# theouterlimitz/Python-Audio-Mastering

Hardware: AMD Instinct MI355X
Metric: stereo frames/sec through full mastering chain, 44.1 kHz f32; 1/2/4/8 GPU (higher is better)
Workload: dtype f64; 1 GPU; C2: 5-min 44.1 kHz stereo f32 track per GPU, full chain (sat 30, techno EQ, width 1.3, multiband defaults, LUFS -14); frames_per_track=13230000, tracks_per_gpu=1, frames_per_rank_step=13230000, parallelism=file-sharded x1, in=f32 interleaved (decoded PCM16), out=f32 interleaved

## Files before the change

### include/mastering.h

```cpp
#ifndef MASTERING_AMD_H
#define MASTERING_AMD_H

#include <stdint.h>

#ifdef __cplusplus
extern "C" {
#endif

#define MM_OK 0
#define MM_ERR_ARG (-1)
#define MM_ERR_HIP (-2)
#define MM_ERR_RCCL (-3)
#define MM_ERR_STATE (-4)

#define MM_MAX_DIM 8
#define MM_TILE_POW 8
#define MM_BLK_POW 65

#define MM_OUT_I16 0
#define MM_OUT_F32 1

#define MM_IN_F32 0
#define MM_IN_I16 1
#define MM_IN_I24 2
// ... 142 lines not shown
    const struct mm_job *loud;
} mm_delivery;

typedef struct mm_solve_geom {
    int32_t tps;
    int32_t tile_rows;
    int32_t rows;
    int32_t walk_block;
    int64_t cols_per_chunk;
    int64_t chunks;
    int64_t chunk_plane_bytes;
    int64_t plane_bytes;
    int32_t col_block;
    int32_t rms_group_tiles;
} mm_solve_geom;

int mm_create(int device, mm_ctx **ctx);
int mm_destroy(mm_ctx *ctx);
const char *mm_last_error(mm_ctx *ctx);
int mm_sync(mm_ctx *ctx);
#define MM_ABI_VERSION 5
int mm_version(void);
int mm_solve_geometry(const mm_job *job, mm_solve_geom *out);
const char *mm_source_sha(void);

int mm_master(mm_ctx *ctx, const mm_job *job, const void *in, void *out, mm_result *res);
int mm_master_device(mm_ctx *ctx, const mm_job *job, const void *d_in, void *d_out, mm_result *res);

#define MM_BATCH_STREAMS 8
int mm_master_batch(mm_ctx *ctx, int n, const mm_job *jobs, const void *const *d_in, void *const *d_out,
                    mm_result *res);

int mm_meter_device(mm_ctx *ctx, const void *d_pcm, int kind, int64_t frames, int channels, const mm_job *loud,
                    mm_meter *out);
int mm_meter_pcm(mm_ctx *ctx, const void *pcm, int kind, int64_t frames, int channels, const mm_job *loud,
                 mm_meter *out);
int mm_last_meters(mm_ctx *ctx, int cap, mm_meter *out);
int mm_true_peak_host(const int16_t *pcm, int64_t frames, int channels, mm_meter *out);
int mm_meter_span(void);

int mm_r128_from_hops(const double *e, int64_t hops, int32_t rate, mm_r128 *out);
int mm_r128_host(const int16_t *pcm, int64_t frames, int channels, int32_t rate, const double sos[2][5],
                 double *hops_out, int64_t hops_cap, mm_r128 *out);
int mm_r128_device(mm_ctx *ctx, const void *d_pcm, int kind, int64_t frames, int channels, int32_t rate,
                   const double sos[2][5], mm_r128 *out);
int mm_r128_pcm(mm_ctx *ctx, const void *pcm, int kind, int64_t frames, int channels, int32_t rate,
// ... 102 lines not shown
```

### python-audio-mastering_amd/csrc/common.h

```cpp
#pragma once
#include <hip/hip_runtime.h>
#include <stdint.h>

#pragma clang fp contract(off)

namespace mm {

__device__ __forceinline__ void lds_barrier() { asm volatile("s_waitcnt lgkmcnt(0)\n\ts_barrier" ::: "memory"); }

__device__ __forceinline__ int32_t pair_swap(int32_t v) { return __builtin_amdgcn_mov_dpp(v, 0xB1, 0xF, 0xF, true); }
__device__ __forceinline__ double pair_swap(double v) {
    const int64_t b = __double_as_longlong(v);
    const int32_t lo = pair_swap((int32_t)(b & 0xffffffff)), hi = pair_swap((int32_t)(b >> 32));
    return __longlong_as_double(((int64_t)hi << 32) | (uint32_t)lo);
}

__device__ __forceinline__ float sqrt_f32_cr(float x) { return (float)__dsqrt_rn((double)x); }

template <int B, int NB, typename V, typename LD, typename PROC>
__device__ __forceinline__ void stream(int len, LD &&ld, PROC &&proc) {
    constexpr int R = B * NB;
    if (len <= 0) return;
    V buf[NB][B];
#pragma unroll
// ... 38 lines not shown
    return true;
}

struct CompArgs {
    int64_t N_proc, G;
    int T, K, ch, warmup;
    int TPS;
    int64_t SPC;
    int64_t GS;
    const short2 *band[3];
    const double *lut[3];
    uint32_t r0[3];
    int look[3];
    double attack_frames[3], release_frames[3];
    double rcp_attack[3], rcp_release[3];
    double *Ms[3];
    int TP;
    int RP;
    int64_t chunk_elems;
    const double *E[3], *tail[3];
    int32_t *cnt[3];
    double *mmax[3];
    double *ced[3];
    int32_t *total[3];
    int32_t *cbtot[3];
    int32_t *rank[3];
    int32_t *nact[3];
    int32_t *tl[3];
    double *mmaxc[3];
    double *cedc[3];
    double *tstc[3];
    double *descc[3];
    double *start[3];
    double *end[3];
    uint32_t *claim[3];
    int jumps;
    int sjump;
    double *sdesc[3];
    int32_t *se0[3];
    uint32_t stamp;
    int heads;
    int e_tiles;
    unsigned int *changed;
    unsigned long long *walked;
    uint32_t *trace;
    int sweep_idx;
// ... 21 lines not shown
```

### python-audio-mastering_amd/csrc/compressor.hip

```cpp
#include "common.h"
#include "lookback.h"

namespace mm {

template <bool V>
struct BoolTag {
    static constexpr bool value = V;
};

__device__ __forceinline__ double div_cr(double m, double d, double rd) {
    const double q = m * rd;
    const double rem = fma(-q, d, m);
    return fma(rem, rd, q);
}

#ifndef MM_RMS_NB
#define MM_RMS_NB 3
#endif
constexpr int RMS_B = 8;
constexpr int RMS_TPS = 4;

__device__ __forceinline__ void tile_col(const CompArgs &a, int64_t g, int64_t *s, int *k) {
    const int64_t c = g / a.K, j = g - c * a.K;
    *s = c * a.SPC + j / a.TPS;
    *k = (int)(j - (j / a.TPS) * a.TPS);
}
__device__ __forceinline__ uint32_t col_elem(const CompArgs &a, int64_t s) {
    const int64_t sl = s % a.SPC;
    return (uint32_t)((sl >> 6) * (int64_t)a.RP * 64 + (sl & 63));
}
__device__ __forceinline__ double *chunk_plane(const CompArgs &a, int b, int64_t c) {
    return a.Ms[b] + c * a.chunk_elems;
}

#ifndef MM_RMS_MINB
#define MM_RMS_MINB 1
#endif
__device__ __forceinline__ uint32_t rms_exact1(double S, double n, float inv_b) {
    int32_t r = (int32_t)__builtin_amdgcn_sqrtf((float)S * inv_b);
    const double rd = (double)(r + 1);
// ... 87 lines not shown
            r = rms_exact1(S, n, inv);
            S += (double)frame_energy2(p.in) - (double)frame_energy2(p.drop);
        } else {
            r = n > 0.0 ? rms_exact1(S, n, inv) : 0u;
            const bool drops = i_proc >= skip;
            S += (double)frame_energy2(p.in) - (drops ? (double)frame_energy2(p.drop) : 0.0);
            if (!drops) {
                n += ch;
                inv = rcp_biased(n);
            }
            ++i_proc;
        }
        active += r >= r0 ? 1 : 0;
        rmx = max(rmx, r);
        return r;
    };
    const int jB = lane & 7;
    const int tlC = lane * 4 + w;
    const int64_t jtC = jt0 + tlC, gC = cc * a.K + jtC;
    const bool vC = jtC < a.K && gC < a.G;
    double *Mo = chunk_plane(a, b, cc);
    uint32_t eC = col_elem(a, cc * a.SPC + jtC / 4) + (uint32_t)(w * a.TP) * 64u;
    double ce = 0.0, De = 0.0;
    const int slotC = w * 68 + lane;

    constexpr int B = RMS_B, NB = MM_RMS_NB;
    const int NBK = (T + B - 1) / B;
    const int NBKP = (NBK + NB - 1) / NB * NB;
    Pair buf[NB][B];
    double gm[B];
#pragma unroll
    for (int j = 0; j < B; ++j) gm[j] = 0.0;
    auto issue_gathers = [&](int q) __attribute__((always_inline)) {
        asm volatile("" ::: "memory");
#pragma unroll
        for (int r8 = 0; r8 < B; ++r8) {
            const int tl = w * 64 + r8 * 8 + (lane >> 3);
            gm[r8] = lut[Rs[q & 1][jB][tl]];
        }
    };
    auto finish_gathers = [&](int q) __attribute__((always_inline)) {
#pragma unroll
        for (int r8 = 0; r8 < B; ++r8) {
            const int tl = w * 64 + r8 * 8 + (lane >> 3);
            Mst[q & 1][jB][rt_slot(tl)] = gm[r8];
        }
    };
    const __amdgpu_buffer_rsrc_t Mr =
        __builtin_amdgcn_make_buffer_rsrc(Mo, (short)0, (int)(a.chunk_elems * 8), 0x00020000);
    constexpr uint32_t DROP = 0xFFFFFFF0u;
    typedef unsigned int u32x2 __attribute__((ext_vector_type(2)));
    auto phase_c = [&](int q) __attribute__((always_inline)) {
        const int nv = q >= 0 ? max(min(B, T - q * B), 0) : 0;
        double m[B];
#pragma unroll
        for (int j = 0; j < B; ++j) m[j] = Mst[q & 1][j][slotC];
#pragma unroll
        for (int j = 0; j < B; ++j) {
            const uint32_t off = (vC && j < nv) ? (eC + (uint32_t)j * 64u) * 8u : DROP;
            __builtin_amdgcn_raw_buffer_store_b64(__builtin_bit_cast(u32x2, m[j]), Mr, off, 0, 0);
        }
        eC += (uint32_t)nv * 64u;
#pragma unroll
        for (int j = 0; j < B; ++j) {
            const double mj = j < nv ? m[j] : 0.0;
            const double d = div_cr(mj, Rf, rR);
            ce = vmax(mj, ce - d);
            De += d;
        }
    };
    auto run = [&](auto st, auto &&load) __attribute__((always_inline)) {
#pragma unroll
        for (int k = 0; k < NB; ++k) {
#pragma unroll
            for (int j = 0; j < B; ++j) buf[k][j] = load(k * B + j);
            __builtin_amdgcn_sched_barrier(0);
        }
        auto body = [&](int k, int q) __attribute__((always_inline)) {
            uint32_t r[B];
            const int nvA = lenA - q * B;
#pragma unroll
            for (int j = 0; j < B; ++j) r[j] = j < nvA ? rms_step(buf[k][j], st) : 0u;
#pragma unroll
            for (int j = 0; j < B; ++j) buf[k][j] = load((q + NB) * B + j);
#pragma unroll
            for (int j = 0; j < B; ++j) Rs[q & 1][j][tlA] = (uint16_t)r[j];
            finish_gathers(q - 1);
            issue_gathers(q);
            __syncthreads();
            phase_c(q - 1);
        };
        for (int q0 = 0; q0 < NBKP; q0 += NB) {
#pragma unroll
            for (int k = 0; k < NB; ++k) body(k, q0 + k);
        }
    };
    if (!__any(vA)) run(BoolTag<true>{}, [](int) { return Pair{make_short2(0, 0), make_short2(0, 0)}; });
    else if (steady) run(BoolTag<true>{}, ld_steady);
    else run(BoolTag<false>{}, ld);
    finish_gathers(NBKP - 1);
    __syncthreads();
    phase_c(NBKP - 1);
    if (vC)
        for (int i = T; i < a.TP; ++i, eC += 64u) Mo[eC] = 0.0;
    if (vC) reinterpret_cast<double2 *>(a.ced[b])[gC] = make_double2(ce, De);
    if (vA) {
        a.cnt[b][gA] = active;
        a.mmax[b][gA] = lut[rmx];
    }
    {
        const int na = (int)__popcll(__ballot(vA && active != 0));
        if (lane == 0 && na) atomicAdd(a.cbtot[b] + cbk, na);
    }
    int v = vA ? active : 0;
    for (int o = 32; o > 0; o >>= 1) v += __shfl_xor(v, o);
    if (lane == 0 && v) atomicAdd(a.total[b] + cc, v);
}

__global__ void __launch_bounds__(64) comp_trim_kernel(CompArgs a, const int64_t *pad) {
    const int b = blockIdx.y, lane = threadIdx.x, T = a.T;
    const int64_t e = pad[2 * blockIdx.x], nx = pad[2 * blockIdx.x + 1];
    int v = 0;
    for (int64_t g = e / T + lane; g < nx / T; g += 64) {
        const int c = a.cnt[b][g];
        const int first = (int)max((int64_t)0, e - g * T);
        if (c == 0) continue;
        if (first == 0) {
            v += c;
// ... 1 lines not shown
        }
        int64_t s;
        int k;
        tile_col(a, g, &s, &k);
        const double *M = chunk_plane(a, b, g / a.K) + col_elem(a, s) + (uint32_t)(k * a.TP) * 64u;
        for (int n = first; n < T; ++n) v += M[(uint32_t)n * 64u] != 0.0 ? 1 : 0;
    }
    for (int o = 32; o > 0; o >>= 1) v += __shfl_xor(v, o);
    if (lane == 0 && v) atomicSub(a.total[b] + (nx / ((int64_t)T * a.K) - 1), v);
}

struct BandStep {
    double A, R, rA, rR;
};

__device__ __forceinline__ BandStep band_step(const CompArgs &a, int b) {
    BandStep s;
    s.A = a.attack_frames[b];
    s.R = a.release_frames[b];
    s.rA = a.rcp_attack[b];
    s.rR = a.rcp_release[b];
    return s;
}

__device__ __forceinline__ int binade(double x) { return (int)((uint64_t)__double_as_longlong(x) >> 52) - 1023; }


__device__ __forceinline__ double vmin(double x, double y) {
    double r;
    asm("v_min_f64 %0, %1, %2" : "=v"(r) : "v"(x), "v"(y));
    return r;
}

__device__ __forceinline__ double lean_step(double att, double m, double inc, double dec) {
    const double up = vmin(att + inc, m);
    const double dn = att - dec;
    return att <= m ? up : dn;
}

struct Super {
    int64_t ci0;
    int ntiles;
    bool first;
    bool last;
};

__device__ __forceinline__ Super super_of_na(const CompArgs &a, int64_t s, int na) {
    Super r;
// ... 109 lines not shown
    BandStep bs;
    double *tst;
    int i0, nst;
    __device__ __forceinline__ void init(const double (&m)[WB]) {
#pragma unroll
        for (int k = 0; k < WP; ++k) {
            inc[k] = div_cr(m[k], bs.A, bs.rA);
            dec[k] = div_cr(m[k], bs.R, bs.rR);
        }
    }
    __device__ __forceinline__ void tile(int i) {
        if (ST && i >= i0 && i < i0 + nst) tst[i - i0] = att;
        if (i == i0) sv = att;
        if (i == i0 + nst) out = att;
    }
    __device__ __forceinline__ void frame(int j, double m, double ma) {
        const double ik = inc[j % WP], dk = dec[j % WP];
        inc[j % WP] = div_cr(ma, bs.A, bs.rA);
        dec[j % WP] = div_cr(ma, bs.R, bs.rR);
        att = lean_step(att, m, ik, dk);
    }
};

#ifndef MM_JB
#define MM_JB 8
#endif
constexpr int JB = MM_JB;
constexpr int JF = JB < 4 ? JB : 4;
struct SegDesc {
    double mx;
    int e0;
    double q[2 * JB];
};
constexpr int DREC = 2 * JB;

__device__ __forceinline__ bool release_jump(const SegDesc &d, double att, double *out) {
    constexpr uint64_t MANT = (1ull << 52) - 1;
    const uint64_t ab = (uint64_t)__double_as_longlong(att);
    const int k = (int)(ab >> 52) - 1023 - d.e0;
    if (!(att > 0.0) || k < 0 || k >= JB) return false;
    const int idx = 2 * k + (int)(ab & 1);
    double q = d.q[0];
#pragma unroll
    for (int j = 1; j < 2 * JB; ++j) q = idx == j ? d.q[j] : q;
    const double x = att - q;
    const uint64_t xb = (uint64_t)__double_as_longlong(x);
    if (!(x > d.mx) || (xb >> 52) != (ab >> 52) || (xb & MANT) == 0) return false;
    *out = x;
    return true;
}

struct Describer {
    static constexpr uint64_t MANT = (1ull << 52) - 1;
    double r0[2 * JB], r[2 * JB];
    int e0;
    BandStep bs;
    __device__ __forceinline__ void init(const double (&)[WB]) {}
    __device__ __forceinline__ void tile(int i) {
        if (i != 0) return;
#pragma unroll
        for (int k = 0; k < 2 * JB; ++k) {
            const uint64_t bits = ((uint64_t)(e0 + k / 2 + 1023) << 52) | (MANT - 63 + (uint64_t)(k % 2));
            r0[k] = r[k] = __longlong_as_double((long long)bits);
        }
    }
    __device__ __forceinline__ void frame(int, double m, double) {
        const double dec = div_cr(m, bs.R, bs.rR);
#pragma unroll
        for (int k = 0; k < 2 * JB; ++k) r[k] = r[k] - dec;
    }
    __device__ __forceinline__ void store(double *rec_) const {
        double2 *rec = reinterpret_cast<double2 *>(rec_);
        double q[2 * JB];
#pragma unroll
        for (int k = 0; k < 2 * JB; ++k) {
            const uint64_t rb = (uint64_t)__double_as_longlong(r[k]);
            const bool ok = (rb >> 52) == (uint64_t)(e0 + k / 2 + 1023) && (rb & MANT) != 0;
            q[k] = ok ? r0[k] - r[k] : __longlong_as_double(0x7ff8000000000000ll);
        }
#pragma unroll
        for (int k = 0; k < JB; ++k) rec[k] = make_double2(q[2 * k], q[2 * k + 1]);
    }
};

#ifndef MM_DESC_NB
#define MM_DESC_NB 1
#endif
constexpr int DESC_MAX_TPS = 8;

__global__ void __launch_bounds__(64 * DESC_MAX_TPS) comp_describe_kernel(CompArgs a) {
    __shared__ int32_t wsum[DESC_MAX_TPS], base_s;
    __shared__ uint8_t flag[64 * DESC_MAX_TPS];
    __shared__ int32_t pre[64 * DESC_MAX_TPS];
    const int b = blockIdx.y;
    const int TPS = a.TPS, NT = 64 * TPS;
    const int kc = threadIdx.x >> 6, l = threadIdx.x & 63;
    const int64_t cb = blockIdx.x;
    const int64_t sc = cb * 64 + l;
    const int64_t cc = sc / a.SPC;
    const int64_t cbl = (sc - cc * a.SPC) >> 6;
    const int64_t jt = (sc - cc * a.SPC) * TPS + kc;
    const int64_t g = cc * a.K + jt;
    const bool valid = jt < a.K && g < a.G;
    const bool live = valid && a.cnt[b][g] != 0;
    flag[l * TPS + kc] = live ? 1 : 0;
    if (threadIdx.x < 64) {
        int32_t acc = 0;
        const int32_t *ct = a.cbtot[b] + cc * (a.SPC >> 6);
        for (int64_t q = threadIdx.x; q < cbl; q += 64) acc += ct[q];
        for (int o = 32; o > 0; o >>= 1) acc += __shfl_xor(acc, o);
        if (threadIdx.x == 0) base_s = acc;
    }
    __syncthreads();
    const int t = threadIdx.x;
    const bool f = flag[t] != 0;
    const uint64_t bal = __ballot(f);
    const int wp = (int)__popcll(bal & ((1ull << (t & 63)) - 1ull));
    if ((t & 63) == 0) wsum[t >> 6] = (int32_t)__popcll(bal);
    __syncthreads();
    int32_t woff = base_s;
    for (int w = 0; w < (t >> 6); ++w) woff += wsum[w];
    pre[t] = woff + wp;
    if (t == NT - 1 && cbl == (a.SPC >> 6) - 1) a.nact[b][cc] = woff + wp + (f ? 1 : 0);
    __syncthreads();
    const int32_t r = pre[l * TPS + kc];
    const int64_t ci = cc * a.K + r;
    if (valid) a.rank[b][g] = r;
    if (live) {
        a.tl[b][ci] = (int32_t)g;
        a.mmaxc[b][ci] = a.mmax[b][g];
        reinterpret_cast<double2 *>(a.cedc[b])[ci] = reinterpret_cast<const double2 *>(a.ced[b])[g];
    }
    if (!a.jumps || __all(!live)) return;
    const int64_t gc = live ? g : cc * a.K;
    Describer d;
    d.bs = band_step(a, b);
    const double mx = a.mmax[b][gc];
    d.e0 = mx > 0.0 ? binade(mx) : 0;
    const uint32_t off = tile_off(a, gc);
    stream_col<true, MM_DESC_NB>(plane(a, b, cc), [&](int) { return off; }, 1, a.TP, d);
    if (live) d.store(a.descc[b] + ci * DREC);
}

constexpr int SJ_TPS = 4;
constexpr int SJ_ENT = SJ_TPS + 1;
#ifndef MM_SJB
#define MM_SJB 4
#endif
constexpr int SJB = MM_SJB < JB ? MM_SJB : JB;
constexpr int SREC = 2 * SJB * SJ_ENT;
constexpr int SJ_NONE = -100000;

__device__ __forceinline__ double next_up(double x) {
    return x > 0.0 ? __longlong_as_double(__double_as_longlong(x) + 1) : x;
}

__device__ void compose_super(const CompArgs &a, int b, int64_t s, int64_t ci0) {
    double mxt[SJ_TPS], q[SJ_TPS][2 * JB];
#pragma unroll
    for (int t = 0; t < SJ_TPS; ++t) {
        mxt[t] = a.mmaxc[b][ci0 + t];
        const double2 *r = reinterpret_cast<const double2 *>(a.descc[b] + (ci0 + t) * DREC);
#pragma unroll
        for (int k = 0; k < JB; ++k) {
            const double2 v = r[k];
            q[t][2 * k] = v.x;
            q[t][2 * k + 1] = v.y;
        }
    }
    double mxs = 0.0;
#pragma unroll
    for (int t = 0; t < SJ_TPS; ++t) mxs = fmax(mxs, mxt[t]);
    const int e0s = binade(mxs);
    double *out = a.sdesc[b] + s * SREC;
#pragma unroll
    for (int k = 0; k < 2 * SJB; ++k) {
        double rec[SJ_ENT];
        double Q = 0.0, L = 0.0;
        int par = k & 1;
        bool ok = true;
        const int e = e0s + k / 2;
#pragma unroll
        for (int t = 0; t < SJ_TPS; ++t) {
            const int kt = e - binade(mxt[t]);
            const int idx = 2 * min(max(kt, 0), JB - 1) + par;
            double qv = q[t][0];
#pragma unroll
            for (int j = 1; j < 2 * JB; ++j) qv = idx == j ? q[t][j] : qv;
            ok = ok && kt >= 0 && kt < JB && qv == qv;
            Q += ok ? qv : 0.0;
            ok = ok && Q < ldexp(1.0, e);
            if (ok) par ^= (int)((int64_t)ldexp(qv, 52 - e) & 1);
            L = fmax(L, next_up(mxt[t] + Q));
            rec[1 + t] = Q;
        }
        rec[0] = ok ? L : __longlong_as_double(0x7ff8000000000000ll);
#pragma unroll
        for (int j = 0; j < SJ_ENT; ++j) out[k * SJ_ENT + j] = rec[j];
    }
    a.se0[b][s] = e0s;
}

template <typename QF>
__device__ __forceinline__ double e_fold_tile(double E, double ct, double Dt, double mx, QF &&qat) {
    constexpr uint64_t MANT = (1ull << 52) - 1;
    if (!(E > 0.0)) return ct;
    const uint64_t ab = (uint64_t)__double_as_longlong(E);
// ... 27 lines not shown
    const Super st = super_of(a, b, sc);
    const bool live = s < a.GS && st.ntiles > 0;
    if (__all(!live)) return;
    const int64_t cK = (sc / a.SPC) * a.K;
    const int W = min(a.warmup, 1);
    const int64_t cw0 = max(cK, st.ci0 - (int64_t)W * a.TPS);
    const int nwarm = live ? (int)(st.ci0 - cw0) : 0, ntot = live ? nwarm + st.ntiles : 0;
    double att = 0.0;
    {
        const int64_t nact_c = a.nact[b][sc / a.SPC];
        const int64_t lo = max(cK, (int64_t)__shfl(cw0, 0) - a.e_tiles);
        const int64_t hi = min(cK + nact_c, (int64_t)__shfl(cw0, 63));
        const int64_t n = hi - lo;
        const bool staged = n <= EW_MAX;
        double *sc_c = reinterpret_cast<double *>(smem);
        double *sc_d = sc_c + EW_MAX, *sc_m = sc_d + EW_MAX, *sc_q = sc_m + EW_MAX;
        if (staged && n > 0) {
            const double2 *cd = reinterpret_cast<const double2 *>(a.cedc[b]);
            const double2 *qd = reinterpret_cast<const double2 *>(a.descc[b]);
            for (int i = lane; i < n; i += PASS0_BLOCK) {
                const double2 v = cd[lo + i];
                sc_c[i] = v.x;
                sc_d[i] = v.y;
                sc_m[i] = a.mmaxc[b][lo + i];
#pragma unroll
                for (int k = 0; k < JF; ++k) {
                    const double2 q = qd[(lo + i) * (DREC / 2) + k];
                    sc_q[(2 * k) * EW_MAX + i] = q.x;
                    sc_q[(2 * k + 1) * EW_MAX + i] = q.y;
                }
            }
        }
        __syncthreads();
        if (live && cw0 != cK && staged) {
            for (int64_t i = max(cK, cw0 - a.e_tiles) - lo; i < cw0 - lo; ++i)
                att = e_fold_tile(att, sc_c[i], sc_d[i], sc_m[i], [&](int idx) { return sc_q[idx * EW_MAX + i]; });
        }
        __syncthreads();
    }
    int nmax = ntot;
    for (int o = 32; o > 0; o >>= 1) nmax = max(nmax, __shfl_xor(nmax, o));
    nmax = __builtin_amdgcn_readfirstlane(nmax);
    const int32_t *tl = a.tl[b];
    for (int i = 0; i < nmax; ++i)
        offs_lds[i][lane] = tile_off(a, ntot ? tl[cw0 + min(i, ntot - 1)] : 0);
    __syncthreads();
    if (a.sjump) {
        if (live && st.ntiles == SJ_TPS && a.TPS == SJ_TPS) compose_super(a, b, s, st.ci0);
        else if (s < a.GS) a.se0[b][s] = SJ_NONE;
    }
// ... 171 lines not shown
                        ring_ok = false;
                        run = next();
                        continue;
                    }
                }
            }
            if (!ring_ok) {
#pragma unroll
                for (int k = 0; k < FIX_AHEAD; ++k) ring[k] = ld(ci + k);
                ring_ok = true;
            }
            m = ring[0];
#pragma unroll
            for (int k = 0; k + 1 < FIX_AHEAD; ++k) ring[k] = ring[k + 1];
            ring[FIX_AHEAD - 1] = ld(ci + FIX_AHEAD);
            if (__double_as_longlong(m.old) == __double_as_longlong(att)) {
                run = false;
                break;
            }
            tst[ci] = att;
            double x;
            SegDesc d;
            d.mx = m.mx;
            d.e0 = binade(m.mx);
#pragma unroll
            for (int k = 0; k < 2 * JB; ++k) d.q[k] = m.q[k];
            if (a.jumps && release_jump(d, att, &x)) {
                att = x;
                jumped += T;
                run = next();
            } else {
                walk = true;
            }
        }
        if (!__any(walk)) break;
        if (walk) {
            Walker<false> w;
            w.att = att;
            w.bs = bs;
            w.i0 = 0;
            w.nst = 1;
            const uint32_t off = tile_off(a, m.g);
            stream_col<true, FIX_WNB>(p, [&](int) { return off; }, 1, a.TP, w);
            att = w.att;
            walked += T;
            walk = false;
            run = next();
// ... 210 lines not shown
```

### python-audio-mastering_amd/csrc/context.h

```cpp
#pragma once

namespace {

struct DevBuf {
    void *p = nullptr;
    size_t cap = 0;
};

struct PendingEvent {
    std::string name;
    hipEvent_t a, b;
};

struct KStat {
    double ms = 0.0;
    int64_t n = 0;
};

struct Solve {
    bool on = false;
    CompArgs ca{};
    uint32_t stamp = 0;
    int iters = 0, pending = 0;
    int queue = 0;
// ... 3 lines not shown
}

struct mm_ctx {
    int device = 0;
    int n_cus = 256;
    hipStream_t stream = nullptr;
    char err[512] = {0};
    std::map<std::string, DevBuf> bufs;
    bool staged = false;
    mm_job job{};
    int64_t G = 0;
    short2 *mix = nullptr;
    ChainCtl ctl;
    Solve comp;
    Loudness loud;
    bool timing = false;
    std::vector<PendingEvent> pending;
    std::vector<hipEvent_t> free_events;
    char *pin[2] = {nullptr, nullptr};
    hipEvent_t pin_ev[2] = {nullptr, nullptr};
    std::map<std::string, KStat> stats;
    std::vector<std::string> stat_order;
    uint64_t lut_key[3] = {0, 0, 0};
    uint64_t sat_key = 0;
    bool sat_codes = false;
    std::map<std::string, std::vector<double>> mats_cache;
    std::vector<mm_ctx *> children;
    std::vector<mm_meter> meters;
    std::vector<mm_r128> r128s;
    std::vector<mm_ceiling> ceilings;
    uint64_t rs_key = 0;
    int rs_L = 0, rs_M = 0, rs_K = 0;
    mm_resample resample{};
    bool resample_valid = false;
    ncclComm_t comm = nullptr;
    int rank = 0, nranks = 1;
};

static int set_err(mm_ctx *c, int code, const char *fmt, ...) {
    if (c) {
        va_list ap;
        va_start(ap, fmt);
        vsnprintf(c->err, sizeof(c->err), fmt, ap);
        va_end(ap);
    }
    return code;
// ... 80 lines not shown
```

### python-audio-mastering_amd/csrc/mastering.hip

```cpp
#include <rccl/rccl.h>

#include <algorithm>
#include <cmath>
#include <cstdarg>
#include <cstdio>
#include <cstring>
#include <map>
#include <string>
#include <vector>

#include "../../include/mastering.h"
#include "iir.hip"
#include "kernels.hip"
#include "compressor.hip"
#include "gate.hip"

using namespace mm;

#include "control.h"
#include "loudness.h"
#include "context.h"
#include "decode.hip"

static int finish_delivered(mm_ctx *c, void *d_out, int kind, int64_t frames, int channels, int i, int32_t ceiling_q28,
// ... 88 lines not shown
    if (j->tiles_per_chunk < 1) return set_err(c, MM_ERR_ARG, "tiles_per_chunk < 1");
    if (j->frames_proc < 0 || j->frames_in < 0) return set_err(c, MM_ERR_ARG, "negative frame count");
    if (j->frames_proc >= (int64_t)1 << 31 || j->frames_in >= (int64_t)1 << 31)
        return set_err(c, MM_ERR_ARG, "track longer than 2^31 frames (32-bit frame indexing)");
    if (j->eq.nsec < 0 || j->eq.nsec > 4) return set_err(c, MM_ERR_ARG, "eq.nsec %d", j->eq.nsec);
    if (j->ceiling_q28 && (j->ceiling_q28 < (1 << 24) || j->ceiling_q28 > (1 << 28)))
        return set_err(c, MM_ERR_ARG, "ceiling_q28 %d out of range [2^24, 2^28]", j->ceiling_q28);
    const int tpb = LB_THREADS / j->channels;
    if (j->eq.nsec > 0 && j->eq.tpb != tpb) return set_err(c, MM_ERR_ARG, "eq tables built for %d tiles/block, need %d", j->eq.tpb, tpb);
    if (j->multiband_on && j->xover.tpb != tpb) return set_err(c, MM_ERR_ARG, "crossover tables built for %d tiles/block", j->xover.tpb);
    if (j->lufs_on && j->kweight.tpb != LB_THREADS) return set_err(c, MM_ERR_ARG, "K-weighting tables built for %d tiles/block", j->kweight.tpb);
    if (j->eq.nsec > 0 && j->eq.tile != j->tile) return set_err(c, MM_ERR_ARG, "eq tables built for %d-frame tiles", j->eq.tile);
    if (j->multiband_on && j->xover.tile != j->tile) return set_err(c, MM_ERR_ARG, "crossover tables built for %d-frame tiles", j->xover.tile);
    if (j->lufs_on && (j->kweight.tile < 1 || j->tile % j->kweight.tile != 0))
        return set_err(c, MM_ERR_ARG, "K-weighting tables built for %d-frame (sub-)tiles, not a divisor of %d",
                       j->kweight.tile, j->tile);
    if (j->multiband_on) {
        if (j->xover.nsec != 4 || j->xover.nsec_branch0 != 2) return set_err(c, MM_ERR_ARG, "crossover must be 2+2 sections");
        for (int b = 0; b < 3; ++b) {
            if (!j->band[b].lut) return set_err(c, MM_ERR_ARG, "band %d: missing table", b);
            if (j->band[b].look < 0) return set_err(c, MM_ERR_ARG, "band %d: look < 0", b);
            if (!(j->band[b].release_frames >= 1.0) || !(j->band[b].attack_frames > 0.0))
                return set_err(c, MM_ERR_ARG, "band %d: release must span >= 1 frame", b);
        }
    }
    if (j->lufs_on) {
        if (j->kweight.nsec != 2) return set_err(c, MM_ERR_ARG, "K-weighting must be 2 sections");
        if (j->n_segs < 1 || !j->seg_bounds || !j->block_lo || !j->block_hi || j->n_blocks < 1)
            return set_err(c, MM_ERR_ARG, "missing loudness geometry");
        for (int64_t s = 0; s < j->n_segs; ++s) {
            int64_t b0 = j->seg_bounds[s], b1 = std::min<int64_t>(j->seg_bounds[s + 1], j->frames_proc);
            if (b1 > b0 && b1 - b0 < j->tile && s + 1 < j->n_segs)
                return set_err(c, MM_ERR_ARG, "loudness segment %lld shorter than a tile", (long long)s);
        }
    }
    return MM_OK;
}

static void fill_sos(double dst[4][5], const mm_iir &f, int n) {
    for (int s = 0; s < 4; ++s)
        for (int k = 0; k < 5; ++k) dst[s][k] = s < n ? f.sos[s][k] : 0.0;
}

template <int NS>
static int launch_eq_ns(mm_ctx *c, int ch, unsigned nblk, const EqArgs &ea, const LbArgs &lb, int64_t K) {
    if (ch == 2) {
// ... 183 lines not shown
    mm_solve_geom sg;
    if (solve_geometry(j, &sg) != MM_OK)
        return set_err(c, MM_ERR_ARG, "chunk of %d tiles too large for one envelope-solve plane", K);
    const int64_t nchunks = sg.chunks;
    ca.TPS = sg.tps;
    ca.SPC = sg.cols_per_chunk;
    ca.GS = nchunks * ca.SPC;
    const int64_t NS = ca.GS;
    short2 *q2;
    RET(get_buf(c, "q2", TG, &q2));
    ca.q_out = q2;
    *q2_out = q2;
    double *st, *ends, *luts, *tstc, *descc, *mmax, *mmaxc, *ced, *cedc;
    RET(get_buf(c, "comp_start", (size_t)3 * NS, &st));
    RET(get_buf(c, "comp_end", (size_t)3 * NS, &ends));
    RET(get_buf(c, "comp_lut", (size_t)3 * 32769, &luts));
    const int64_t NC = nchunks * K;
    RET(get_buf(c, "comp_mmax", (size_t)3 * G, &mmax));
    RET(get_buf(c, "comp_tstc", (size_t)3 * NC, &tstc));
    RET(get_buf(c, "comp_mmaxc", (size_t)3 * NC, &mmaxc));
    RET(get_buf(c, "comp_ced", (size_t)6 * G, &ced));
    RET(get_buf(c, "comp_cedc", (size_t)6 * NC, &cedc));
    RET(get_buf(c, "comp_descc", (size_t)3 * DREC * NC, &descc));
    int32_t *ranks, *tls, *nacts;
    RET(get_buf(c, "comp_rank", (size_t)3 * G, &ranks));
    RET(get_buf(c, "comp_tl", (size_t)3 * NC, &tls));
    RET(get_buf(c, "comp_nact", (size_t)3 * nchunks, &nacts));
    ca.jumps = getenv("MM_COMP_NOJUMP") ? 0 : 1;
    ca.sjump = ca.jumps && !getenv("MM_COMP_NOSJUMP") && ca.TPS == SJ_TPS ? 1 : 0;
    ca.e_tiles = E_TILES;
    double *sdesc;
    int32_t *se0s;
    RET(get_buf(c, "comp_sdesc", ca.sjump ? (size_t)3 * NS * SREC : 1, &sdesc));
    RET(get_buf(c, "comp_se0", ca.sjump ? (size_t)3 * NS : 1, &se0s));
    ca.walked = c->ctl.dev()->walked;
    ca.trace = nullptr;
    if (getenv("MM_FIX_TRACE")) {
        RET(get_buf(c, "comp_trace", (size_t)16 * 3 * NS * 4, &ca.trace));
        HIPCHK(c, hipMemsetAsync(ca.trace, 0, (size_t)16 * 3 * NS * 4 * sizeof(uint32_t), c->stream));
    }
    ca.TP = sg.tile_rows;
    ca.RP = sg.rows;
    ca.chunk_elems = sg.chunk_plane_bytes / 8;
    const int64_t ms_elems = ca.chunk_elems * nchunks;
    int32_t *cnt;
    RET(get_buf(c, "comp_cnt", (size_t)3 * G, &cnt));
// ... 10 lines not shown
        if (j->band[b].lut_key == 0 || c->lut_key[b] != j->band[b].lut_key) {
            HIPCHK(c, hipMemcpy2DAsync(luts + (size_t)b * 32769, sizeof(double), j->band[b].lut,
                                       4 * sizeof(double), sizeof(double), 32769, hipMemcpyHostToDevice,
                                       c->stream));
            c->lut_key[b] = j->band[b].lut_key;
        }
        ca.r0[b] = (uint32_t)j->band[b].r0;
        ca.look[b] = j->band[b].look;
        ca.attack_frames[b] = j->band[b].attack_frames;
        ca.release_frames[b] = j->band[b].release_frames;
        ca.rcp_attack[b] = 1.0 / j->band[b].attack_frames;
        ca.rcp_release[b] = 1.0 / j->band[b].release_frames;
        ca.cnt[b] = cnt + (size_t)b * G;
        ca.mmax[b] = mmax + (size_t)b * G;
        ca.total[b] = c->ctl.dev_totals(b);
        ca.rank[b] = ranks + (size_t)b * G;
        ca.nact[b] = nacts + (size_t)b * nchunks;
        ca.tl[b] = tls + (size_t)b * NC;
        ca.mmaxc[b] = mmaxc + (size_t)b * NC;
        ca.ced[b] = ced + (size_t)2 * b * G;
        ca.cedc[b] = cedc + (size_t)2 * b * NC;
        ca.tstc[b] = tstc + (size_t)b * NC;
        ca.descc[b] = descc + (size_t)b * DREC * NC;
        ca.start[b] = st + (size_t)b * NS;
        ca.end[b] = ends + (size_t)b * NS;
        ca.claim[b] = c->ctl.claims(b);
        ca.sdesc[b] = ca.sjump ? sdesc + (size_t)b * NS * SREC : nullptr;
        ca.se0[b] = ca.sjump ? se0s + (size_t)b * NS : nullptr;
        ca.cbtot[b] = c->ctl.cbtot(b);
    }
    RET(launch(c, "comp_rms", comp_rms_t_kernel, dim3((unsigned)(NS / 64), 3), dim3(256), 0, ca));
    if (n_pad > 0)
        RET(launch(c, "comp_trim", comp_trim_kernel, dim3((unsigned)n_pad, 3), dim3(64), 0, ca, pad));
    RET(launch(c, "comp_describe", comp_describe_kernel, dim3((unsigned)(NS / 64), 3), dim3(64 * ca.TPS), 0, ca));
    RET(launch(c, "comp_pass0", comp_pass0_kernel, dim3(blocks_for(NS, PASS0_BLOCK), 3), dim3(PASS0_BLOCK), 0, ca));
    Solve &sv = c->comp;
    sv.on = true;
    sv.ca = ca;
    sv.stamp = 0;
    sv.iters = sv.pending = 0;
    const uint64_t sig = comp_signature(j);
    if (sig != sv.sig) {
        sv.queue = 0;
        sv.sig = sig;
    }
    int sweeps = sv.queue > 0 ? sv.queue : COMP_SWEEPS;
// ... 430 lines not shown
                while (k < i + run - (parts - q - 1) && acc + padded(k) / 2 <= goal) acc += padded(k++);
            }
            Unit u = unit(first, k - first);
            if (u.n > 1 && !unit_layout(&u)) {
                for (int t = first; t < k; ++t) units.push_back(unit(t, 1));
                continue;
            }
            units.push_back(std::move(u));
        }
        i += run;
    }
    return units;
}

extern "C" {

int mm_version(void) { return MM_ABI_VERSION; }

int mm_solve_geometry(const mm_job *j, mm_solve_geom *out) {
    if (!j || !out) return MM_ERR_ARG;
    return solve_geometry(j, out);
}

#ifndef MM_SOURCE_SHA
#define MM_SOURCE_SHA "unknown"
#endif
const char *mm_source_sha(void) { return MM_SOURCE_SHA; }

int mm_create(int device, mm_ctx **out) {
    if (!out) return MM_ERR_ARG;
    *out = nullptr;
    mm_ctx *c = new mm_ctx();
    c->device = device;
    if (hipSetDevice(device) != hipSuccess) {
        delete c;
        return MM_ERR_HIP;
    }
    if (hipStreamCreateWithFlags(&c->stream, hipStreamNonBlocking) != hipSuccess) {
        delete c;
        return MM_ERR_HIP;
    }
    int ncu = 0;
    if (hipDeviceGetAttribute(&ncu, hipDeviceAttributeMultiprocessorCount, device) == hipSuccess && ncu > 0)
        c->n_cus = ncu;
    *out = c;
    return MM_OK;
// ... 175 lines not shown
```

### python-audio-mastering_amd/mastering_amd/native.py

```python
from __future__ import annotations

import ctypes
import os
import threading

_HERE = os.path.dirname(os.path.abspath(__file__))
LIB_PATH = os.environ.get("MM_LIB") or os.path.join(_HERE, "libmastering_amd.so")

MM_OUT_I16, MM_OUT_F32 = 0, 1
MM_IN_F32, MM_IN_I16 = 0, 1
MM_IN_I24, MM_IN_I32 = 2, 3
MM_F32, MM_F64 = 0, 1
MM_ERR_ARG = -1
BATCH_STREAMS = 8
MAX_DIM, TILE_POW, BLK_POW = 8, 8, 65

c_double_p = ctypes.POINTER(ctypes.c_double)
c_int64_p = ctypes.POINTER(ctypes.c_int64)


class MMIir(ctypes.Structure):
    _fields_ = [("nsec", ctypes.c_int32), ("nsec_branch0", ctypes.c_int32), ("dim", ctypes.c_int32),
                ("tpb", ctypes.c_int32), ("tile", ctypes.c_int32), ("_pad", ctypes.c_int32),
                ("sos", (ctypes.c_double * 5) * 4),
# ... 81 lines not shown
    _fields_ = [("rs", ctypes.POINTER(MMResampler)), ("ceiling_q28", ctypes.c_int32), ("window", ctypes.c_int32),
                ("meter_on", ctypes.c_int32), ("_pad", ctypes.c_int32), ("loud", ctypes.POINTER(MMJob))]


ABI_VERSION = 5


class MMWavInfo(ctypes.Structure):
    _fields_ = [("frames", ctypes.c_int64), ("data_offset", ctypes.c_int64), ("rate", ctypes.c_int32),
                ("channels", ctypes.c_int32), ("format", ctypes.c_int32), ("bits", ctypes.c_int32)]


EXPORTS = ("mm_create", "mm_destroy", "mm_last_error", "mm_sync", "mm_version", "mm_source_sha", "mm_master",
           "mm_master_device",
           "mm_stage_chunks", "mm_kweight_range_end", "mm_hop_energies", "mm_shard_loudness_device",
           "mm_shard_energies_device", "mm_gate_finalize_device", "mm_allreduce_sum_f64_device",
           "mm_allgather_f64_device",
           "mm_gate_loudness", "mm_finalize",
           "mm_read_mix", "mm_timing", "mm_kernel_stats", "mm_comm_unique_id", "mm_comm_init", "mm_comm_destroy",
           "mm_allreduce_sum_f64", "mm_allgather_f64", "mm_wav_probe", "mm_master_wav",
           "mm_op_pcm_to_float", "mm_op_saturation", "mm_op_saturation_table", "mm_op_stereo_width", "mm_op_quantize", "mm_op_soft_limiter",
           "mm_op_gain", "mm_op_sosfilt", "mm_op_loudness", "mm_op_multiband", "mm_master_batch",
           "mm_op_saturation_legacy", "mm_op_soft_limiter_legacy", "mm_op_sosfilt_mix", "mm_op_compress_bands",
           "mm_solve_geometry", "mm_np_sum_f32", "mm_check_compressor_math",
           "mm_meter_device", "mm_meter_pcm", "mm_last_meters", "mm_op_true_peak", "mm_true_peak_host",
           "mm_meter_span",
           "mm_r128_from_hops", "mm_r128_host", "mm_r128_device", "mm_r128_pcm", "mm_op_r128_hops", "mm_r128_span",
           "mm_last_r128",
           "mm_ceiling_device", "mm_ceiling_pcm", "mm_ceiling_host", "mm_last_ceilings", "mm_ceiling_span",
           "mm_ceiling_max_window",
           "mm_pcm_decode_device", "mm_op_pcm_decode", "mm_pcm_decode_host", "mm_pcm_decode_span",
           "mm_resample_device", "mm_resample_pcm", "mm_resample_host", "mm_resample_frames", "mm_resample_span",
           "mm_last_resample", "mm_deliver_device", "mm_deliver", "mm_deliver_wav")

_lib = None
_lock = threading.Lock()


def load():
    global _lib
    with _lock:
        if _lib is not None:
            return _lib
        try:
            import torch
        except Exception:
            pass
# ... 36 lines not shown
            "mm_comm_destroy": ([vp], ctypes.c_int),
            "mm_allreduce_sum_f64": ([vp, c_double_p, ctypes.c_int64], ctypes.c_int),
            "mm_allgather_f64": ([vp, c_double_p, c_double_p, ctypes.c_int64], ctypes.c_int),
            "mm_allreduce_sum_f64_device": ([vp, vp, ctypes.c_int64], ctypes.c_int),
            "mm_allgather_f64_device": ([vp, vp, vp, ctypes.c_int64], ctypes.c_int),
            "mm_op_pcm_to_float": ([vp, vp, ctypes.c_int64, vp], ctypes.c_int),
            "mm_op_saturation": ([vp, ctypes.c_int, vp, ctypes.c_int64, ctypes.c_double, vp], ctypes.c_int),
            "mm_op_saturation_table": ([vp, ctypes.c_int, vp, ctypes.c_int64, ctypes.c_double,
                                        ctypes.POINTER(ctypes.c_float), vp], ctypes.c_int),
            "mm_op_stereo_width": ([vp, ctypes.c_int, vp, ctypes.c_int64, ctypes.c_double, vp], ctypes.c_int),
            "mm_op_quantize": ([vp, ctypes.c_int, vp, ctypes.c_int64, vp], ctypes.c_int),
            "mm_op_soft_limiter": ([vp, ctypes.c_int, vp, ctypes.c_int64, ctypes.c_double], ctypes.c_int),
            "mm_op_gain": ([vp, ctypes.c_int, vp, ctypes.c_int64, ctypes.c_double, vp], ctypes.c_int),
            "mm_op_sosfilt": ([vp, ctypes.c_int, vp, ctypes.c_int64, ctypes.c_int, P(MMIir), ctypes.c_int, vp],
                              ctypes.c_int),
            "mm_op_loudness": ([vp, P(MMJob), ctypes.c_int, vp, c_double_p], ctypes.c_int),
            "mm_op_multiband": ([vp, P(MMJob), vp, vp], ctypes.c_int),
            "mm_op_saturation_legacy": ([vp, ctypes.c_int, vp, ctypes.c_int64, ctypes.c_double, vp], ctypes.c_int),
            "mm_op_soft_limiter_legacy": ([vp, ctypes.c_int, vp, ctypes.c_int64, ctypes.c_double], ctypes.c_int),
            "mm_op_sosfilt_mix": ([vp, ctypes.c_int, vp, ctypes.c_int64, ctypes.c_int, P(MMIir), ctypes.c_double,
                                   ctypes.c_double, vp], ctypes.c_int),
            "mm_op_compress_bands": ([vp, P(MMJob), vp, vp, vp, vp], ctypes.c_int),
            "mm_solve_geometry": ([P(MMJob), P(MMSolveGeom)], ctypes.c_int),
            "mm_np_sum_f32": ([P(ctypes.c_float), ctypes.c_int64, P(ctypes.c_float)], ctypes.c_int),
            "mm_check_compressor_math": ([vp, ctypes.c_int, c_double_p, c_double_p, ctypes.c_int64, c_double_p],
                                         ctypes.c_int),
            "mm_meter_device": ([vp, vp, ctypes.c_int, ctypes.c_int64, ctypes.c_int, P(MMJob), P(MMMeter)],
                                ctypes.c_int),
            "mm_meter_pcm": ([vp, vp, ctypes.c_int, ctypes.c_int64, ctypes.c_int, P(MMJob), P(MMMeter)],
                             ctypes.c_int),
            "mm_last_meters": ([vp, ctypes.c_int, P(MMMeter)], ctypes.c_int),
            "mm_op_true_peak": ([vp, ctypes.c_int, vp, ctypes.c_int64, ctypes.c_int, c_double_p], ctypes.c_int),
            "mm_true_peak_host": ([P(ctypes.c_int16), ctypes.c_int64, ctypes.c_int, P(MMMeter)], ctypes.c_int),
            "mm_meter_span": ([], ctypes.c_int),
            "mm_r128_from_hops": ([c_double_p, ctypes.c_int64, ctypes.c_int32, P(MMR128)], ctypes.c_int),
            "mm_r128_host": ([P(ctypes.c_int16), ctypes.c_int64, ctypes.c_int, ctypes.c_int32, c_sos_p, c_double_p,
                              ctypes.c_int64, P(MMR128)], ctypes.c_int),
            "mm_r128_device": ([vp, vp, ctypes.c_int, ctypes.c_int64, ctypes.c_int, ctypes.c_int32, c_sos_p,
                                P(MMR128)], ctypes.c_int),
            "mm_r128_pcm": ([vp, vp, ctypes.c_int, ctypes.c_int64, ctypes.c_int, ctypes.c_int32, c_sos_p,
                             P(MMR128)], ctypes.c_int),
            "mm_op_r128_hops": ([vp, vp, ctypes.c_int, ctypes.c_int64, ctypes.c_int, ctypes.c_int32, c_sos_p,
                                 c_double_p, ctypes.c_int64], ctypes.c_int),
            "mm_r128_span": ([], ctypes.c_int),
            "mm_last_r128": ([vp, ctypes.c_int, P(MMR128)], ctypes.c_int),
            "mm_ceiling_device": ([vp, vp, ctypes.c_int, ctypes.c_int64, ctypes.c_int, ctypes.c_int32, ctypes.c_int32,
# ... 95 lines not shown
```

Before: 11.71 billion stereo frames/s.

## Fuse jump-descriptor records into RMS pass using fixed binade base

The RMS/envelope kernel now builds release-jump descriptor records for each tile as it runs, against a fixed exponent base derived from the LUT's top value. The compact kernel then only re-streams tiles whose max falls below that base, and copies the precomputed records for the rest. The aim is to avoid a second pass over the envelope plane for most live tiles. In exchange the RMS loop carries 16 extra subtractions per frame and more registers, with the prefetch depth knob dropped from 3 to 1. It also adds a host-side validation of the LUT's r0 and a debug export of the records.

```diff
diff --git a/include/mastering.h b/include/mastering.h
--- a/include/mastering.h
+++ b/include/mastering.h
@@ -188,6 +188,8 @@
 #define MM_ABI_VERSION 5
 int mm_version(void);
 int mm_solve_geometry(const mm_job *job, mm_solve_geom *out);
+int mm_solve_records(mm_ctx *ctx, int band, int64_t cap, int32_t *tiles, double *mmax, double *records,
+                     int64_t *count);
 const char *mm_source_sha(void);
 
 int mm_master(mm_ctx *ctx, const mm_job *job, const void *in, void *out, mm_result *res);
diff --git a/python-audio-mastering_amd/csrc/common.h b/python-audio-mastering_amd/csrc/common.h
--- a/python-audio-mastering_amd/csrc/common.h
+++ b/python-audio-mastering_amd/csrc/common.h
@@ -84,6 +84,8 @@
     int32_t *cnt[3];
     double *mmax[3];
     double *ced[3];
+    int e0fix[3];
+    double *desc_g[3];
     int32_t *total[3];
     int32_t *cbtot[3];
     int32_t *rank[3];
diff --git a/python-audio-mastering_amd/csrc/compressor.hip b/python-audio-mastering_amd/csrc/compressor.hip
--- a/python-audio-mastering_amd/csrc/compressor.hip
+++ b/python-audio-mastering_amd/csrc/compressor.hip
@@ -14,8 +14,31 @@
     return fma(rem, rd, q);
 }
 
+__device__ __forceinline__ int binade(double x) { return (int)((uint64_t)__double_as_longlong(x) >> 52) - 1023; }
+
+#ifndef MM_JB
+#define MM_JB 8
+#endif
+constexpr int JB = MM_JB;
+constexpr int JF = JB < 4 ? JB : 4;
+constexpr int DREC = 2 * JB;
+__device__ __forceinline__ int rec_base(double mx, int e0fix) {
+    const int e = binade(mx);
+    return e >= e0fix ? e0fix : e;
+}
+__device__ __forceinline__ double ref_start(int e, int p) {
+    constexpr uint64_t MANT = (1ull << 52) - 1;
+    return __longlong_as_double((long long)(((uint64_t)(e + 1023) << 52) | (MANT - 63 + (uint64_t)p)));
+}
+__device__ __forceinline__ double ref_entry(int e, int p, double r) {
+    constexpr uint64_t MANT = (1ull << 52) - 1;
+    const uint64_t rb = (uint64_t)__double_as_longlong(r);
+    const bool ok = (rb >> 52) == (uint64_t)(e + 1023) && (rb & MANT) != 0;
+    return ok ? ref_start(e, p) - r : __longlong_as_double(0x7ff8000000000000ll);
+}
+
 #ifndef MM_RMS_NB
-#define MM_RMS_NB 3
+#define MM_RMS_NB 1
 #endif
 constexpr int RMS_B = 8;
 constexpr int RMS_TPS = 4;
@@ -149,7 +172,12 @@
     double *Mo = chunk_plane(a, b, cc);
     uint32_t eC = col_elem(a, cc * a.SPC + jtC / 4) + (uint32_t)(w * a.TP) * 64u;
     double ce = 0.0, De = 0.0;
+    bool anyM = false;
     const int slotC = w * 68 + lane;
+    const int e0f = a.e0fix[b];
+    double ref[2 * JB];
+#pragma unroll
+    for (int k = 0; k < 2 * JB; ++k) ref[k] = ref_start(e0f + k / 2, k % 2);
 
     constexpr int B = RMS_B, NB = MM_RMS_NB;
     const int NBK = (T + B - 1) / B;
@@ -194,6 +222,9 @@
             const double d = div_cr(mj, Rf, rR);
             ce = vmax(mj, ce - d);
             De += d;
+            anyM = anyM || mj != 0.0;
+#pragma unroll
+            for (int k = 0; k < 2 * JB; ++k) ref[k] = ref[k] - d;
         }
     };
     auto run = [&](auto st, auto &&load) __attribute__((always_inline)) {
@@ -231,6 +262,12 @@
     if (vC)
         for (int i = T; i < a.TP; ++i, eC += 64u) Mo[eC] = 0.0;
     if (vC) reinterpret_cast<double2 *>(a.ced[b])[gC] = make_double2(ce, De);
+    if (vC && anyM) {
+        double2 *rec = reinterpret_cast<double2 *>(a.desc_g[b] + gC * DREC);
+#pragma unroll
+        for (int k = 0; k < JB; ++k)
+            rec[k] = make_double2(ref_entry(e0f + k, 0, ref[2 * k]), ref_entry(e0f + k, 1, ref[2 * k + 1]));
+    }
     if (vA) {
         a.cnt[b][gA] = active;
         a.mmax[b][gA] = lut[rmx];
@@ -278,8 +315,6 @@
     s.rR = a.rcp_release[b];
     return s;
 }
-
-__device__ __forceinline__ int binade(double x) { return (int)((uint64_t)__double_as_longlong(x) >> 52) - 1023; }
 
 
 __device__ __forceinline__ double vmin(double x, double y) {
@@ -435,17 +470,11 @@
     }
 };
 
-#ifndef MM_JB
-#define MM_JB 8
-#endif
-constexpr int JB = MM_JB;
-constexpr int JF = JB < 4 ? JB : 4;
 struct SegDesc {
     double mx;
     int e0;
     double q[2 * JB];
 };
-constexpr int DREC = 2 * JB;
 
 __device__ __forceinline__ bool release_jump(const SegDesc &d, double att, double *out) {
     constexpr uint64_t MANT = (1ull << 52) - 1;
@@ -464,18 +493,14 @@
 }
 
 struct Describer {
-    static constexpr uint64_t MANT = (1ull << 52) - 1;
-    double r0[2 * JB], r[2 * JB];
+    double r[2 * JB];
     int e0;
     BandStep bs;
     __device__ __forceinline__ void init(const double (&)[WB]) {}
     __device__ __forceinline__ void tile(int i) {
         if (i != 0) return;
 #pragma unroll
-        for (int k = 0; k < 2 * JB; ++k) {
-            const uint64_t bits = ((uint64_t)(e0 + k / 2 + 1023) << 52) | (MANT - 63 + (uint64_t)(k % 2));
-            r0[k] = r[k] = __longlong_as_double((long long)bits);
-        }
+        for (int k = 0; k < 2 * JB; ++k) r[k] = ref_start(e0 + k / 2, k % 2);
     }
     __device__ __forceinline__ void frame(int, double m, double) {
         const double dec = div_cr(m, bs.R, bs.rR);
@@ -484,15 +509,9 @@
     }
     __device__ __forceinline__ void store(double *rec_) const {
         double2 *rec = reinterpret_cast<double2 *>(rec_);
-        double q[2 * JB];
-#pragma unroll
-        for (int k = 0; k < 2 * JB; ++k) {
-            const uint64_t rb = (uint64_t)__double_as_longlong(r[k]);
-            const bool ok = (rb >> 52) == (uint64_t)(e0 + k / 2 + 1023) && (rb & MANT) != 0;
-            q[k] = ok ? r0[k] - r[k] : __longlong_as_double(0x7ff8000000000000ll);
-        }
-#pragma unroll
-        for (int k = 0; k < JB; ++k) rec[k] = make_double2(q[2 * k], q[2 * k + 1]);
+#pragma unroll
+        for (int k = 0; k < JB; ++k)
+            rec[k] = make_double2(ref_entry(e0 + k, 0, r[2 * k]), ref_entry(e0 + k, 1, r[2 * k + 1]));
     }
 };
 
@@ -516,7 +535,9 @@
     const int64_t g = cc * a.K + jt;
     const bool valid = jt < a.K && g < a.G;
     const bool live = valid && a.cnt[b][g] != 0;
-    flag[l * TPS + kc] = live ? 1 : 0;
+    const double mx = live ? a.mmax[b][g] : 0.0;
+    const bool own = live && binade(mx) < a.e0fix[b];
+    flag[l * TPS + kc] = live ? (own ? 1 : 3) : 0;
     if (threadIdx.x < 64) {
         int32_t acc = 0;
         const int32_t *ct = a.cbtot[b] + cc * (a.SPC >> 6);
@@ -544,15 +565,24 @@
         a.mmaxc[b][ci] = a.mmax[b][g];
         reinterpret_cast<double2 *>(a.cedc[b])[ci] = reinterpret_cast<const double2 *>(a.ced[b])[g];
     }
-    if (!a.jumps || __all(!live)) return;
-    const int64_t gc = live ? g : cc * a.K;
+    if (!a.jumps) return;
+    {
+        const double2 *__restrict__ src = reinterpret_cast<const double2 *>(a.desc_g[b]) + (g - (l * TPS + kc)) * JB;
+        double2 *__restrict__ dst = reinterpret_cast<double2 *>(a.descc[b]) + cc * a.K * JB;
+#pragma unroll
+        for (int it = 0; it < JB; ++it) {
+            const int e = it * NT + t, i = e / JB;
+            if (flag[i] == 3) dst[(int64_t)pre[i] * JB + (e - i * JB)] = src[e];
+        }
+    }
+    if (__all(!own)) return;
+    const int64_t gc = own ? g : cc * a.K;
     Describer d;
     d.bs = band_step(a, b);
-    const double mx = a.mmax[b][gc];
-    d.e0 = mx > 0.0 ? binade(mx) : 0;
+    d.e0 = own ? binade(mx) : 0;
     const uint32_t off = tile_off(a, gc);
     stream_col<true, MM_DESC_NB>(plane(a, b, cc), [&](int) { return off; }, 1, a.TP, d);
-    if (live) d.store(a.descc[b] + ci * DREC);
+    if (own) d.store(a.descc[b] + ci * DREC);
 }
 
 constexpr int SJ_TPS = 4;
@@ -595,7 +625,7 @@
         const int e = e0s + k / 2;
 #pragma unroll
         for (int t = 0; t < SJ_TPS; ++t) {
-            const int kt = e - binade(mxt[t]);
+            const int kt = e - rec_base(mxt[t], a.e0fix[b]);
             const int idx = 2 * min(max(kt, 0), JB - 1) + par;
             double qv = q[t][0];
 #pragma unroll
@@ -669,10 +699,13 @@
                 const double2 v = cd[lo + i];
                 sc_c[i] = v.x;
                 sc_d[i] = v.y;
-                sc_m[i] = a.mmaxc[b][lo + i];
+                const double mxi = a.mmaxc[b][lo + i];
+                sc_m[i] = mxi;
+                const int sh = binade(mxi) - rec_base(mxi, a.e0fix[b]);
 #pragma unroll
                 for (int k = 0; k < JF; ++k) {
-                    const double2 q = qd[(lo + i) * (DREC / 2) + k];
+                    const double nan = __longlong_as_double(0x7ff8000000000000ll);
+                    const double2 q = sh + k < JB ? qd[(lo + i) * (DREC / 2) + sh + k] : make_double2(nan, nan);
                     sc_q[(2 * k) * EW_MAX + i] = q.x;
                     sc_q[(2 * k + 1) * EW_MAX + i] = q.y;
                 }
@@ -890,7 +923,7 @@
             double x;
             SegDesc d;
             d.mx = m.mx;
-            d.e0 = binade(m.mx);
+            d.e0 = rec_base(m.mx, a.e0fix[b]);
 #pragma unroll
             for (int k = 0; k < 2 * JB; ++k) d.q[k] = m.q[k];
             if (a.jumps && release_jump(d, att, &x)) {
diff --git a/python-audio-mastering_amd/csrc/context.h b/python-audio-mastering_amd/csrc/context.h
--- a/python-audio-mastering_amd/csrc/context.h
+++ b/python-audio-mastering_amd/csrc/context.h
@@ -49,6 +49,8 @@
     std::map<std::string, KStat> stats;
     std::vector<std::string> stat_order;
     uint64_t lut_key[3] = {0, 0, 0};
+    uint64_t lut_ok_key[3] = {0, 0, 0};
+    int64_t lut_ok_r0[3] = {0, 0, 0};
     uint64_t sat_key = 0;
     bool sat_codes = false;
     std::map<std::string, std::vector<double>> mats_cache;
diff --git a/python-audio-mastering_amd/csrc/mastering.hip b/python-audio-mastering_amd/csrc/mastering.hip
--- a/python-audio-mastering_amd/csrc/mastering.hip
+++ b/python-audio-mastering_amd/csrc/mastering.hip
@@ -134,6 +134,17 @@
             if (j->band[b].look < 0) return set_err(c, MM_ERR_ARG, "band %d: look < 0", b);
             if (!(j->band[b].release_frames >= 1.0) || !(j->band[b].attack_frames > 0.0))
                 return set_err(c, MM_ERR_ARG, "band %d: release must span >= 1 frame", b);
+            const double *lt = j->band[b].lut;
+            const int64_t r0 = j->band[b].r0;
+            const uint64_t key = j->band[b].lut_key;
+            bool ok = r0 >= 0 && r0 <= 32769 && (r0 == 0 || lt[4 * (r0 - 1)] == 0.0) &&
+                      (r0 > 32768 || lt[4 * r0] != 0.0);
+            if (ok && (key == 0 || c->lut_ok_key[b] != key || c->lut_ok_r0[b] != r0)) {
+                for (int64_t r = 0; r <= 32768 && ok; ++r) ok = (lt[4 * r] != 0.0) == (r >= r0);
+                c->lut_ok_key[b] = ok ? key : 0;
+                c->lut_ok_r0[b] = r0;
+            }
+            if (!ok) return set_err(c, MM_ERR_ARG, "band %d: r0 %lld is not the table's first nonzero row", b, (long long)r0);
         }
     }
     if (j->lufs_on) {
@@ -363,6 +374,8 @@
     RET(get_buf(c, "comp_ced", (size_t)6 * G, &ced));
     RET(get_buf(c, "comp_cedc", (size_t)6 * NC, &cedc));
     RET(get_buf(c, "comp_descc", (size_t)3 * DREC * NC, &descc));
+    double *desc_g;
+    RET(get_buf(c, "comp_desc_g", (size_t)3 * DREC * std::max<int64_t>(G, 1), &desc_g));
     int32_t *ranks, *tls, *nacts;
     RET(get_buf(c, "comp_rank", (size_t)3 * G, &ranks));
     RET(get_buf(c, "comp_tl", (size_t)3 * NC, &tls));
@@ -419,6 +432,9 @@
         ca.cedc[b] = cedc + (size_t)2 * b * NC;
         ca.tstc[b] = tstc + (size_t)b * NC;
         ca.descc[b] = descc + (size_t)b * DREC * NC;
+        ca.desc_g[b] = desc_g + (size_t)b * DREC * G;
+        const double mtop = j->band[b].lut[(size_t)4 * 32768];
+        ca.e0fix[b] = (mtop > 0.0 ? std::max(ilogb(mtop), -900) : 0) - (JB - 1);
         ca.start[b] = st + (size_t)b * NS;
         ca.end[b] = ends + (size_t)b * NS;
         ca.claim[b] = c->ctl.claims(b);
@@ -895,6 +911,34 @@
     return solve_geometry(j, out);
 }
 
+int mm_solve_records(mm_ctx *c, int band, int64_t cap, int32_t *tiles, double *mmax, double *records,
+                     int64_t *count) {
+    if (!c || !count || band < 0 || band > 2 || cap < 0 || (cap > 0 && (!tiles || !mmax || !records)))
+        return set_err(c, MM_ERR_ARG, "bad arguments");
+    const Solve &sv = c->comp;
+    if (!sv.on) return set_err(c, MM_ERR_STATE, "no envelope solve on this context");
+    const CompArgs &ca = sv.ca;
+    HIPCHK(c, hipSetDevice(c->device));
+    HIPCHK(c, hipStreamSynchronize(c->stream));
+    const int64_t nchunks = ca.GS / ca.SPC;
+    std::vector<int32_t> nact((size_t)nchunks);
+    HIPCHK(c, hipMemcpy(nact.data(), ca.nact[band], (size_t)nchunks * sizeof(int32_t), hipMemcpyDeviceToHost));
+    int64_t n = 0;
+    for (int64_t ch = 0; ch < nchunks; ++ch) {
+        const int64_t na = nact[(size_t)ch], take = std::max<int64_t>(0, std::min(na, cap - n));
+        const int64_t ci = ch * ca.K;
+        if (take > 0) {
+            HIPCHK(c, hipMemcpy(tiles + n, ca.tl[band] + ci, (size_t)take * sizeof(int32_t), hipMemcpyDeviceToHost));
+            HIPCHK(c, hipMemcpy(mmax + n, ca.mmaxc[band] + ci, (size_t)take * sizeof(double), hipMemcpyDeviceToHost));
+            HIPCHK(c, hipMemcpy(records + n * DREC, ca.descc[band] + ci * DREC, (size_t)take * DREC * sizeof(double),
+                                hipMemcpyDeviceToHost));
+        }
+        n += na;
+    }
+    *count = n;
+    return MM_OK;
+}
+
 #ifndef MM_SOURCE_SHA
 #define MM_SOURCE_SHA "unknown"
 #endif
diff --git a/python-audio-mastering_amd/mastering_amd/native.py b/python-audio-mastering_amd/mastering_amd/native.py
--- a/python-audio-mastering_amd/mastering_amd/native.py
+++ b/python-audio-mastering_amd/mastering_amd/native.py
@@ -127,7 +127,7 @@
            "mm_op_pcm_to_float", "mm_op_saturation", "mm_op_saturation_table", "mm_op_stereo_width", "mm_op_quantize", "mm_op_soft_limiter",
            "mm_op_gain", "mm_op_sosfilt", "mm_op_loudness", "mm_op_multiband", "mm_master_batch",
            "mm_op_saturation_legacy", "mm_op_soft_limiter_legacy", "mm_op_sosfilt_mix", "mm_op_compress_bands",
-           "mm_solve_geometry", "mm_np_sum_f32", "mm_check_compressor_math",
+           "mm_solve_geometry", "mm_solve_records", "mm_np_sum_f32", "mm_check_compressor_math",
            "mm_meter_device", "mm_meter_pcm", "mm_last_meters", "mm_op_true_peak", "mm_true_peak_host",
            "mm_meter_span",
            "mm_r128_from_hops", "mm_r128_host", "mm_r128_device", "mm_r128_pcm", "mm_op_r128_hops", "mm_r128_span",
@@ -210,6 +210,8 @@
                                    ctypes.c_double, vp], ctypes.c_int),
             "mm_op_compress_bands": ([vp, P(MMJob), vp, vp, vp, vp], ctypes.c_int),
             "mm_solve_geometry": ([P(MMJob), P(MMSolveGeom)], ctypes.c_int),
+            "mm_solve_records": ([vp, ctypes.c_int, ctypes.c_int64, P(ctypes.c_int32), c_double_p, c_double_p,
+                                  c_int64_p], ctypes.c_int),
             "mm_np_sum_f32": ([P(ctypes.c_float), ctypes.c_int64, P(ctypes.c_float)], ctypes.c_int),
             "mm_check_compressor_math": ([vp, ctypes.c_int, c_double_p, c_double_p, ctypes.c_int64, c_double_p],
                                          ctypes.c_int),
```

Result: faster. 12.00 billion stereo frames/s, median of 6 (+2.4%).
